# teboli/polyblur

Hardware: AMD Instinct MI355X
Metric: megapixels/sec (n_iter=3, alpha=6, beta=1) (higher is better)
Workload: dtype f32; 1 GPU; batch=1 3840x2160x3 fp32 per GPU, n_iter=3, method=fft (circular), full 25-tap support; mode=resident, images_per_gpu=1, height=2160, width=3840, parallelism=images sharded, no data-path collective

## Files before the change

include/polyblur_hip.h:

```cpp
#ifndef POLYBLUR_HIP_H
#define POLYBLUR_HIP_H

#include <stddef.h>
#include <stdint.h>

#ifdef __cplusplus
extern "C" {
#endif

#define PB_VERSION 200
#define PB_KSIZE 25
#define PB_KRAD 12
#define PB_MAX_ANGLES 13
#define PB_MAX_INTERP 64
#define PB_MAX_PHASES 175

typedef struct pb_ctx pb_ctx;

typedef enum pb_status {
    PB_OK = 0,
    PB_ERR_BADARG = -1,
    PB_ERR_UNSUPPORTED = -2,
    PB_ERR_HIP = -3,
    PB_ERR_NOMEM = -4
// ... 43 lines not shown
    float kx[PB_KSIZE], ky[PB_KSIZE];
    float acorr_y[PB_KSIZE], acorr_x[PB_KSIZE];
    float gtaps[(PB_KSIZE + 1) * 32];
    float gtaps_odd[(PB_KSIZE + 1) * 32];
    int32_t xt_first;
    int32_t xt_exact_rank1;
    float xt_g1[PB_KSIZE];
    int32_t xt_m[PB_KSIZE];
    float xt_wa[PB_KSIZE], xt_wb[PB_KSIZE];
    int32_t nphase[3];
    int32_t phase[PB_MAX_PHASES + 9];
} pb_blur_info;

int pb_version(void);
int pb_create(pb_ctx **out, int device, void *stream);
int pb_destroy(pb_ctx *ctx);
int pb_set_stream(pb_ctx *ctx, void *stream);
int pb_synchronize(pb_ctx *ctx);
const char *pb_last_error_string(pb_ctx *ctx);
void pb_default_options(pb_options *opt);
typedef enum pb_dense_eval { PB_DENSE_STENCIL = 0, PB_DENSE_AUTO = 1 } pb_dense_eval;
int pb_set_dense_eval(pb_ctx *ctx, int mode, int min_phases);
int pb_body_selection(pb_ctx *ctx, int iteration, int *host, int B);
size_t pb_workspace_bytes(pb_ctx *ctx);

int pb_malloc(pb_ctx *ctx, void **dptr, size_t bytes);
int pb_free(pb_ctx *ctx, void *dptr);
int pb_memcpy_h2d(pb_ctx *ctx, void *dst, const void *src, size_t bytes);
int pb_memcpy_d2h(pb_ctx *ctx, void *dst, const void *src, size_t bytes);

int pb_polyblur_batch(pb_ctx *ctx, const void *in, void *out, int dtype,
                      int B, int C, int H, int W, const pb_options *opt,
                      pb_blur_info *host_info);

int pb_u8_deinterleave(pb_ctx *ctx, const unsigned char *hwc, unsigned char *chw, int B, int C, int H, int W);
int pb_u8_interleave(pb_ctx *ctx, const unsigned char *chw, unsigned char *hwc, int B, int C, int H, int W);


int pb_estimate_blur(pb_ctx *ctx, const void *in, int dtype, int B, int C, int H, int W,
                     const pb_options *opt, pb_blur_info *dev_info);

int pb_make_kernels(pb_ctx *ctx, int B, const float *host_sigma, const float *host_rho,
                    const float *host_theta_rad, int support, pb_blur_info *dev_info);
int pb_set_kernels(pb_ctx *ctx, int B, const float *host_taps, int support, pb_blur_info *dev_info);

int pb_make_separable_kernels(pb_ctx *ctx, int B, const pb_blur_info *dev_info, pb_blur_info *dev_sep, int support,
// ... 77 lines not shown
```

polyblur_amd/_capi.py:

```python
from __future__ import annotations

import ctypes as C
import os
import threading

import numpy as np

PB_KSIZE = 25
PB_KSIZE_MAX = 49
PB_MAX_ANGLES = 13
PB_MAX_INTERP = 64
PB_MAX_PHASES = 175

PB_F32, PB_F16, PB_U8 = 0, 1, 2
PB_WRAP, PB_ZERO = 0, 1
PB_PREFILTER_NONE, PB_PREFILTER_BILATERAL, PB_PREFILTER_DOMAIN_TRANSFORM, PB_PREFILTER_NORMALIZED_CONVOLUTION = 0, 1, 2, 3
PB_SUPPORT_FULL, PB_SUPPORT_ADAPTIVE = 0, 1
PB_DENSE_STENCIL, PB_DENSE_AUTO = 0, 1
PB_DENSE_MIN_PHASES = 16
PB_COMM_CHUNK_AUTO = -1

STATUS = {0: "PB_OK", -1: "PB_ERR_BADARG", -2: "PB_ERR_UNSUPPORTED", -3: "PB_ERR_HIP", -4: "PB_ERR_NOMEM"}

SYMBOLS = [
    "pb_version", "pb_create", "pb_destroy", "pb_set_stream", "pb_synchronize", "pb_last_error_string",
    "pb_default_options", "pb_workspace_bytes", "pb_malloc", "pb_free", "pb_memcpy_h2d", "pb_memcpy_d2h",
    "pb_polyblur_batch", "pb_estimate_blur", "pb_make_kernels", "pb_set_kernels", "pb_fourier_gradients",
    "pb_inverse_filter", "pb_convolve2d", "pb_edgetaper", "pb_halo_mask", "pb_dt_recursive_filter",
    "pb_bilateral5", "pb_time_inner_loop", "pb_profile_begin", "pb_profile_end", "pb_extract_patches",
    "pb_overlap_add", "pb_u8_deinterleave", "pb_u8_interleave", "pb_dt_normalized_convolution",
    "pb_fft_length_supported", "pb_make_separable_kernels", "pb_set_dense_eval",
    "pb_body_selection",
    "pb_comm_shard", "pb_comm_unique_id", "pb_comm_init", "pb_comm_destroy", "pb_comm_scatter", "pb_comm_gather",
    "pb_comm_deblur_from_root", "pb_comm_plan_steps", "pb_comm_plan", "pb_comm_set_chunk", "pb_comm_default_chunk",
    "pb_comm_plan_steps_chunked", "pb_comm_plan_chunked",
]
PROF_TAGS = ["conv", "gray", "grad_rows", "grad_cols", "params", "halo", "prefilter", "other", "conv_fused", "conv_fft"]


class pb_options(C.Structure):
    _fields_ = [
        ("n_iter", C.c_int32), ("c", C.c_float), ("b", C.c_float), ("alpha", C.c_float), ("beta", C.c_float),
        ("sigma_s", C.c_float), ("sigma_r", C.c_float), ("q", C.c_float), ("n_angles", C.c_int32),
        ("n_interpolated_angles", C.c_int32), ("remove_halo", C.c_int32), ("edgetaping", C.c_int32),
        ("prefilter", C.c_int32), ("discard_saturation", C.c_int32), ("boundary", C.c_int32),
        ("support", C.c_int32), ("force_theta_deg", C.c_float), ("separable_approx", C.c_int32), ("half_temporaries", C.c_int32), ("ker_size", C.c_int32),
    ]


class pb_blur_info(C.Structure):
    _fields_ = [
        ("gray_min", C.c_float), ("gray_max", C.c_float), ("mags", C.c_float * PB_MAX_ANGLES),
        ("interp", C.c_float * PB_MAX_INTERP), ("i_min", C.c_int32), ("theta", C.c_float),
        ("sigma", C.c_float), ("rho", C.c_float), ("separable", C.c_int32), ("radius", C.c_int32),
        ("kernel", C.c_float * (PB_KSIZE * PB_KSIZE)), ("kx", C.c_float * PB_KSIZE), ("ky", C.c_float * PB_KSIZE),
# ... 58 lines not shown
            "pb_free": (ci, [vp, vp]),
            "pb_memcpy_h2d": (ci, [vp, vp, vp, sz]),
            "pb_memcpy_d2h": (ci, [vp, vp, vp, sz]),
            "pb_polyblur_batch": (ci, [vp, vp, vp, ci, ci, ci, ci, ci, C.POINTER(pb_options), vp]),
            "pb_u8_deinterleave": (ci, [vp, vp, vp, ci, ci, ci, ci]),
            "pb_u8_interleave": (ci, [vp, vp, vp, ci, ci, ci, ci]),
            "pb_estimate_blur": (ci, [vp, vp, ci, ci, ci, ci, ci, C.POINTER(pb_options), vp]),
            "pb_make_kernels": (ci, [vp, ci, fp, fp, fp, ci, vp]),
            "pb_set_kernels": (ci, [vp, ci, fp, ci, vp]),
            "pb_fourier_gradients": (ci, [vp, vp, ci, ci, ci, vp, vp]),
            "pb_inverse_filter": (ci, [vp, vp, vp, ci, ci, ci, ci, ci, vp, cf, cf, ci, ci, ci, vp, vp]),
            "pb_convolve2d": (ci, [vp, vp, vp, ci, ci, ci, ci, vp, ci]),
            "pb_edgetaper": (ci, [vp, vp, vp, ci, ci, ci, ci, vp, ci]),
            "pb_halo_mask": (ci, [vp, vp, vp, vp, vp, vp, ci, ci, ci, ci]),
            "pb_dt_recursive_filter": (ci, [vp, vp, vp, vp, ci, ci, ci, ci, ci, cf, cf, ci]),
            "pb_dt_normalized_convolution": (ci, [vp, vp, vp, ci, ci, ci, ci, ci, cf, cf, ci]),
            "pb_bilateral5": (ci, [vp, vp, vp, ci, ci, ci, ci, ci]),
            "pb_time_inner_loop": (ci, [vp, vp, vp, ci, ci, ci, ci, ci, vp, cf, cf, ci, ci, fp]),
            "pb_extract_patches": (ci, [vp, vp, vp] + [ci] * 15),
            "pb_overlap_add": (ci, [vp, vp, vp] + [ci] * 13 + [vp, vp]),
            "pb_fft_length_supported": (ci, [ci]),
            "pb_make_separable_kernels": (ci, [vp, ci, vp, vp, ci, ci]),
            "pb_body_selection": (ci, [vp, ci, C.POINTER(ci), ci]),
            "pb_profile_begin": (ci, [vp]),
            "pb_profile_end": (ci, [vp, fp, C.POINTER(ci)]),
            "pb_comm_shard": (ci, [ci, ci, ci, C.POINTER(ci), C.POINTER(ci)]),
            "pb_comm_unique_id": (ci, [C.c_char_p]),
            "pb_comm_init": (ci, [C.POINTER(vp), vp, ci, ci, C.c_char_p]),
            "pb_comm_destroy": (ci, [vp]),
            "pb_comm_scatter": (ci, [vp, vp, vp, ci, ci, ci, ci, ci, ci]),
            "pb_comm_gather": (ci, [vp, vp, vp, ci, ci, ci, ci, ci, ci]),
            "pb_comm_deblur_from_root": (ci, [vp, vp, vp, ci, ci, ci, ci, ci, C.POINTER(pb_options), ci]),
            "pb_comm_plan_steps": (ci, [ci, ci, ci]),
            "pb_comm_plan": (ci, [ci, ci, ci, ci, ci, C.POINTER(ci), C.POINTER(ci)]),
            "pb_comm_set_chunk": (ci, [vp, ci]),
            "pb_comm_default_chunk": (ci, [ci, ci, ci]),
            "pb_comm_plan_steps_chunked": (ci, [ci, ci, ci, ci]),
            "pb_comm_plan_chunked": (ci, [ci, ci, ci, ci, ci, ci, C.POINTER(ci), C.POINTER(ci)]),
        }
        for name in SYMBOLS:
            fn = getattr(lib, name)
            fn.restype, fn.argtypes = proto[name]
        _lib = lib
        return lib
```

polyblur_amd/csrc/api.hip:

```cpp
#include <cstdlib>
#include <cstring>

#include "common.h"

int pb_grad_energy(pb_ctx *ctx, const void *gx, const void *gy, float *nM, int P, long HW, int g_dtype = PB_F32);
int pb_halo_apply(pb_ctx *ctx, const void *x, int x_dtype, int x_pitch, long x_plane, const float *y, const void *gx,
                  const void *gy, const void *ox, const float *nM, void *out, int out_dtype, int P, int H, int W,
                  int clamp01, const void *recomb_cur = nullptr, int recomb_cur_dtype = 0, const float *recomb_smooth = nullptr,
                  int g_dtype = PB_F32);
int pb_recombine(pb_ctx *ctx, const float *y, const void *cur, int cur_dtype, const float *smooth, void *out, int out_dtype,
                 long n);
int pb_bilateral5_impl(pb_ctx *ctx, const void *in, int in_dtype, void *out, int out_dtype, int P, int H, int W);
int pb_dt_filter_impl(pb_ctx *ctx, const void *in, const void *joint, int dtype, float *out, int B, int C, int H, int W,
                      float sigma_s, float sigma_r, int num_iterations);
int pb_nc_filter_impl(pb_ctx *ctx, const void *in, int dtype, float *out, int B, int C, int H, int W, float sigma_s,
                      float sigma_r, int num_iterations);
int pb_convert_from_float(pb_ctx *ctx, const float *in, void *out, int dtype, long n);
int pb_u8_layout(pb_ctx *ctx, const unsigned char *in, unsigned char *out, int B, int C, int H, int W, int to_planar);
int pb_convert_to_float(pb_ctx *ctx, const void *in, int dtype, float *out, long n);
int pb_extract_patches_impl(pb_ctx *ctx, const void *img, void *patches, int dtype, int B, int C, int H, int W, int ph, int pw,
                            int step_h, int step_w, int n_j, int pad_top, int pad_left, int first, int count);
int pb_overlap_add_impl(pb_ctx *ctx, const void *patches, void *out, int dtype, int B, int C, int H, int W, int ph, int pw,
                        int step_h, int step_w, int n_i, int n_j, int pad_top, int pad_left, const float *win_y,
                        const float *win_x);
// ... 56 lines not shown
}

extern "C" {

int pb_version(void) { return PB_VERSION; }

void pb_default_options(pb_options *o) {
    memset(o, 0, sizeof(*o));
    o->n_iter = 1; o->c = 0.352f; o->b = 0.768f; o->alpha = 2.f; o->beta = 3.f;
    o->sigma_r = 0.8f; o->sigma_s = 2.0f; o->q = 0.f; o->n_angles = 6; o->n_interpolated_angles = 30;
    o->remove_halo = 0; o->edgetaping = 0; o->prefilter = PB_PREFILTER_NONE; o->discard_saturation = 0;
    o->boundary = PB_WRAP; o->support = PB_SUPPORT_FULL; o->force_theta_deg = -1.f; o->ker_size = PB_KSIZE;
}

int pb_create(pb_ctx **out, int device, void *stream) {
    if (!out) return PB_ERR_BADARG;
    *out = nullptr;
    int n = 0;
    if (hipGetDeviceCount(&n) != hipSuccess || n <= 0 || device < 0 || device >= n) return PB_ERR_HIP;
    if (hipSetDevice(device) != hipSuccess) return PB_ERR_HIP;
    pb_ctx *ctx = new pb_ctx();
    ctx->device = device;
    ctx->stream = static_cast<hipStream_t>(stream);
    pb_read_knobs(ctx);
    if (hipEventCreate(&ctx->ev0) != hipSuccess || hipEventCreate(&ctx->ev1) != hipSuccess ||
        hipEventCreateWithFlags(&ctx->ev_switch, hipEventDisableTiming) != hipSuccess) { delete ctx; return PB_ERR_HIP; }
    {
        if (hipStreamCreateWithFlags(&ctx->aux, hipStreamNonBlocking) != hipSuccess ||
            hipEventCreateWithFlags(&ctx->ev_fork, hipEventDisableTiming) != hipSuccess ||
            hipEventCreateWithFlags(&ctx->ev_join, hipEventDisableTiming) != hipSuccess) {
            (void)hipGetLastError();
            if (ctx->aux) (void)hipStreamDestroy(ctx->aux);
            ctx->aux = nullptr;
        }
    }
    *out = ctx;
    return PB_OK;
}

int pb_set_dense_eval(pb_ctx *ctx, int mode, int min_phases) {
    if (!ctx || (mode != PB_DENSE_STENCIL && mode != PB_DENSE_AUTO) || min_phases < 0 || min_phases > PB_MAX_PHASES + 1)
        return PB_ERR_BADARG;
    ctx->fft_min_phases = mode == PB_DENSE_STENCIL ? -1 : min_phases;
    pb_forget_records(ctx, nullptr, 0);
    return PB_OK;
}
// ... 811 lines not shown
```

polyblur_amd/csrc/common.h:

```cpp
#pragma once
#include <hip/hip_runtime.h>
#include <hip/hip_fp16.h>

#include <cstdarg>
#include <cstdio>
#include <map>
#include <string>
#include <vector>

#include "../../include/polyblur_hip.h"


struct FftPlan {
    int n = 0;
    int nstage = 0;
    int radix[24];
    int bluestein_m = 0;
    float2 *tw = nullptr;
    float *drev = nullptr;
    float2 *chirp = nullptr;
    float2 *bfilt_rev = nullptr;
    float *dnat = nullptr;
};

// ... 1 lines not shown
    void *p = nullptr;
    size_t bytes = 0;
};

struct ProfRec {
    hipEvent_t a, b;
    int tag;
};

struct PolySpec { int on; float a3, a2, a1, b; float gain; int min_area; float cost128; int always; };
inline PolySpec no_poly() { return PolySpec{0, 0.f, 0.f, 0.f, 0.f, 0.f, 0, 0.f, 0}; }
inline bool same_spec(const PolySpec &x, const PolySpec &y) {
    return x.on == y.on && x.always == y.always &&
           (!x.on || (x.a3 == y.a3 && x.a2 == y.a2 && x.a1 == y.a1 && x.b == y.b && (x.cost128 > 0.f) == (y.cost128 > 0.f)));
}

struct pb_fft_sel { int use_fft; int rf; int strip; int poly; int hx; int hy; int pad_[2]; };

struct pb_ctx {
    bool prof_on = false;
    std::vector<ProfRec> prof;
    std::vector<hipEvent_t> evpool;
    int device = 0;
    hipStream_t stream = nullptr;
    std::string err;
    std::map<std::string, ScratchBuf> scratch;
    std::map<int, FftPlan> plans;
    float *interp_w = nullptr;
    int interp_na = 0, interp_ni = 0;
    hipEvent_t ev0 = nullptr, ev1 = nullptr, ev_switch = nullptr;
    hipStream_t aux = nullptr;
    hipEvent_t ev_fork = nullptr, ev_join = nullptr;
    size_t est_done_bytes = 0;
    int fft_min_phases = 16;
    int fft_wave = 1;
    struct BodyFlags { bool any_fft = false, any_other = false, any_strip = false, any_tile = false, any_fft3 = false; };
    struct RecFlags { int B; BodyFlags plain; bool poly_valid; PolySpec spec; BodyFlags poly; std::vector<pb_fft_sel> sel; };
    std::map<const void *, RecFlags> rec_cache;
    struct FlipSet { int B; int support; std::vector<float> taps; };
    std::map<const void *, FlipSet> flip_sets;
    int sel_slot = 0, sel_last = 0, sel_B = 0;
    const std::vector<pb_fft_sel> *known_sel = nullptr;
    const void *khat_owner = nullptr;
    int khat_slot = 0;
    int khat_B = 0;
    const void *khat_buf = nullptr;
// ... 181 lines not shown
```

polyblur_amd/csrc/conv_w128.hip:

```cpp

#include <algorithm>
#include <cstdlib>
#include <type_traits>

#include "conv_wave_common.h"

namespace {

constexpr int W_N = 128;
constexpr int W_P = 129;
constexpr size_t kW128Lds = sizeof(float2) * 64 * W_P;

static __device__ const float kC128[64] = {
    1.0f, 0.9987954497337341f, 0.9951847195625305f, 0.9891765117645264f, 0.9807852506637573f, 0.9700312614440918f,
    0.9569403529167175f, 0.9415440559387207f, 0.9238795042037964f, 0.903989315032959f, 0.8819212913513184f, 0.8577286005020142f,
    0.8314695954322815f, 0.803207516670227f, 0.7730104327201843f, 0.7409511208534241f, 0.7071067690849304f, 0.6715589761734009f,
    0.6343932747840881f, 0.5956993103027344f, 0.5555702447891235f, 0.5141027569770813f, 0.4713967442512512f, 0.4275550842285156f,
    0.3826834261417389f, 0.3368898630142212f, 0.290284663438797f, 0.24298018217086792f, 0.19509032368659973f, 0.1467304676771164f,
    0.0980171412229538f, 0.049067676067352295f, 6.123234262925839e-17f, -0.049067676067352295f, -0.0980171412229538f, -0.1467304676771164f,
    -0.19509032368659973f, -0.24298018217086792f, -0.290284663438797f, -0.3368898630142212f, -0.3826834261417389f, -0.4275550842285156f,
    -0.4713967442512512f, -0.5141027569770813f, -0.5555702447891235f, -0.5956993103027344f, -0.6343932747840881f, -0.6715589761734009f,
    -0.7071067690849304f, -0.7409511208534241f, -0.7730104327201843f, -0.803207516670227f, -0.8314695954322815f, -0.8577286005020142f,
    -0.8819212913513184f, -0.903989315032959f, -0.9238795042037964f, -0.9415440559387207f, -0.9569403529167175f, -0.9700312614440918f,
    -0.9807852506637573f, -0.9891765117645264f, -0.9951847195625305f, -0.9987954497337341f};
// ... 352 lines not shown
            const int row0 = 64 * h;
            const int rlo = max(hy - row0, 0), rhi = min(rmax - row0, 64);
            const unsigned baseA = okA && rlo < rhi ? (unsigned)((wy0 + row0 + rlo - oo) * opitchb + (pxA - oo) * (int)sizeof(TOut)) : kNoAccess;
            const unsigned baseB = okB && rlo < rhi ? (unsigned)((wy0 + row0 + rlo - oo) * opitchb + (pxB - oo) * (int)sizeof(TOut)) : kNoAccess;
#pragma unroll
            for (int r = 0; r < 64; ++r) {
                const bool rok = r >= rlo && r < rhi;
                cf ea = v[r], eb = v[r];
                swap_halves(ea, eb);
                const cf er = ea + eb * sg;
                const float ra = __builtin_amdgcn_fmed3f(er.x, clo, chi), rb = __builtin_amdgcn_fmed3f(er.y, clo, chi);
                BufIO<TOut>::st(ro, rok ? baseA + (unsigned)((r - rlo) * opitchb) : kNoAccess, 0, ra);
                BufIO<TOut>::st(ro, rok ? baseB + (unsigned)((r - rlo) * opitchb) : kNoAccess, 0, rb);
            }
        }
    }
    PB_WT(8);
    PB_WRT(10);
}

template <typename TIn, typename TOut, bool ZERO>
__global__ __launch_bounds__(256, 2) void conv_w128_kernel(const ConvPass a, const W128Geom g) {
    extern __shared__ __attribute__((aligned(16))) float2 Zw[];
    const int lane = threadIdx.x & 63;
#if defined(PB_EXPERIMENTAL) && defined(PB_W128_TRACE)
    unsigned long long *tr = (blockIdx.x < kTraceGroups && threadIdx.x < 64) ? g_w128_trace + (long)blockIdx.x * kTraceStamps : nullptr;
    PB_WT(0);
    PB_WRT(9);
#endif
    const int C = a.C, B = a.P / C;
    const int q = (int)(blockIdx.x & 7u);
    int rem = (int)(blockIdx.x >> 3);
    int img = 0, hx = 0, hy = 0;
    if (B == 1) {
        const PB_CONSTANT pb_fft_sel *s0 = as_constant(a.fsel);
        if (!s0->use_fft || s0->poly != 2) return;
        hx = s0->hx; hy = s0->hy;
    } else {
        auto share_of = [&](int i) -> int {
            if (i >= B) return 0;
            const pb_fft_sel s = a.fsel[i];
            if (!s.use_fft || s.poly != 2) return 0;
            return jobs128_of(g, s.hx, s.hy).per * C;
        };
        bool work = false;
        int base = 0;
        for (int c0 = 0; c0 < B; c0 += 64) {
            const int n = share_of(c0 + lane), incl = wave_scan(n, lane);
            const unsigned long long m = __ballot(base + incl > rem);
            if (m) {
                const int l = __builtin_ctzll(m);
                img = c0 + l;
                rem -= base + (__builtin_amdgcn_readlane(incl, l) - __builtin_amdgcn_readlane(n, l));
                work = true;
                break;
            }
            base += __builtin_amdgcn_readlane(incl, 63);
        }
        if (!work) return;
        img = __builtin_amdgcn_readfirstlane(img); rem = __builtin_amdgcn_readfirstlane(rem);
        hx = as_constant(a.fsel + img)->hx; hy = as_constant(a.fsel + img)->hy;
    }
    const W128Jobs j = jobs128_of(g, hx, hy);
    const int pl = __builtin_amdgcn_readfirstlane(div_rcp128(rem, __builtin_amdgcn_rcpf((float)j.per)));
    if (pl >= C) return;
    const int pair = q * j.per + (rem - pl * j.per);
    if (pair >= j.njobs) return;
    const int ty = __builtin_amdgcn_readfirstlane(div_rcp128(pair, j.inv_pairs_x)), pxi = pair - ty * j.pairs_x;
    w128_pair<TIn, TOut, ZERO>(a, img * C + pl, ty, pxi, hx, hy, Zw, a.khat + (long)img * PB_KHAT_STRIDE PB_WT_PASS);
}

template <typename TIn, typename TOut>
int launch_w128_typed(pb_ctx *ctx, const ConvPass &p, const W128Geom &g, long groups) {
    if (p.boundary == PB_ZERO)
        hipLaunchKernelGGL((conv_w128_kernel<TIn, TOut, true>), dim3((unsigned)groups), dim3(256), kW128Lds, ctx->stream, p, g);
    else
        hipLaunchKernelGGL((conv_w128_kernel<TIn, TOut, false>), dim3((unsigned)groups), dim3(256), kW128Lds, ctx->stream, p, g);
    PB_LAUNCH_CHECK();
    return PB_OK;
}

}

#if defined(PB_EXPERIMENTAL) && defined(PB_W128_TRACE)
extern "C" int pb_debug_w128_trace(unsigned long long *host) {
    int rc = (int)hipMemcpyFromSymbol(host, HIP_SYMBOL(g_w128_trace), sizeof(g_w128_trace));
    static unsigned long long zeros[kTraceGroups * kTraceStamps];
    if (!rc) rc = (int)hipMemcpyToSymbol(HIP_SYMBOL(g_w128_trace), zeros, sizeof(zeros));
    return rc;
}
#endif

bool pb_conv_w128_types(int in_dtype, int out_dtype) { return in_dtype >= 0 && in_dtype <= 2 && out_dtype >= 0 && out_dtype <= 2; }

bool pb_conv_w128_feasible(const ConvPass &p) {
    const int oh = (p.out_kind == OUT_INTERIOR) ? p.H : p.H + 2 * p.pad, ow = (p.out_kind == OUT_INTERIOR) ? p.W : p.W + 2 * p.pad;
    const int t = PB_POLY128_MIN_T;
    const long nj = (long)(((ow + t - 1) / t + 1) / 2) * ((oh + t - 1) / t);
    const long groups = 8L * ((nj + 7) / 8) * p.P;
    return groups > 0 && groups <= (1L << 23);
// ... 41 lines not shown
```

polyblur_amd/csrc/conv_wave_common.h:

```cpp
#pragma once
#include "conv_fft_common.h"

namespace {

constexpr int WF_ROWS = 32;
constexpr size_t kWfLdsWave = sizeof(float2) * WF_ROWS * FT_P;

static __device__ const float kC64[64] = {
    1.0f, 0.9951847195625305f, 0.9807852506637573f, 0.9569403529167175f, 0.9238795042037964f, 0.8819212913513184f,
    0.8314695954322815f, 0.7730104327201843f, 0.7071067690849304f, 0.6343932747840881f, 0.5555702447891235f,
    0.4713967442512512f, 0.3826834261417389f, 0.290284663438797f, 0.19509032368659973f, 0.0980171412229538f, 0.0f,
    -0.0980171412229538f, -0.19509032368659973f, -0.290284663438797f, -0.3826834261417389f, -0.4713967442512512f,
    -0.5555702447891235f, -0.6343932747840881f, -0.7071067690849304f, -0.7730104327201843f, -0.8314695954322815f,
    -0.8819212913513184f, -0.9238795042037964f, -0.9569403529167175f, -0.9807852506637573f, -0.9951847195625305f, -1.0f,
    -0.9951847195625305f, -0.9807852506637573f, -0.9569403529167175f, -0.9238795042037964f, -0.8819212913513184f,
    -0.8314695954322815f, -0.7730104327201843f, -0.7071067690849304f, -0.6343932747840881f, -0.5555702447891235f,
    -0.4713967442512512f, -0.3826834261417389f, -0.290284663438797f, -0.19509032368659973f, -0.0980171412229538f, 0.0f,
    0.0980171412229538f, 0.19509032368659973f, 0.290284663438797f, 0.3826834261417389f, 0.4713967442512512f,
    0.5555702447891235f, 0.6343932747840881f, 0.7071067690849304f, 0.7730104327201843f, 0.8314695954322815f,
    0.8819212913513184f, 0.9238795042037964f, 0.9569403529167175f, 0.9807852506637573f, 0.9951847195625305f};
static __device__ const float kS64[64] = {
    0.0f, 0.0980171412229538f, 0.19509032368659973f, 0.290284663438797f, 0.3826834261417389f, 0.4713967442512512f,
    0.5555702447891235f, 0.6343932747840881f, 0.7071067690849304f, 0.7730104327201843f, 0.8314695954322815f,
    0.8819212913513184f, 0.9238795042037964f, 0.9569403529167175f, 0.9807852506637573f, 0.9951847195625305f, 1.0f,
// ... 89 lines not shown
__device__ __forceinline__ void swap_halves(cf &hi_part, cf &lo_part) {
    typedef unsigned u2 __attribute__((ext_vector_type(2)));
    const u2 x = __builtin_amdgcn_permlane32_swap(__float_as_uint(hi_part.x), __float_as_uint(lo_part.x), false, false);
    const u2 y = __builtin_amdgcn_permlane32_swap(__float_as_uint(hi_part.y), __float_as_uint(lo_part.y), false, false);
    hi_part = (cf){__uint_as_float(x[0]), __uint_as_float(y[0])};
    lo_part = (cf){__uint_as_float(x[1]), __uint_as_float(y[1])};
}

__device__ __forceinline__ void transpose64(cf (&v)[64], float2 *Z, int lane) {
#pragma unroll
    for (int r = 0; r < 32; ++r) swap_halves(v[r], v[32 + r]);
    const float2 *rd = Z + (lane & 31) * FT_P + (lane & 32);
#pragma unroll
    for (int h = 0; h < 2; ++h) {
#pragma unroll
        for (int r = 0; r < 32; ++r) Z[r * FT_P + lane] = pbfft::to_f2(v[32 * h + r]);
        wave_lds_fence();
#pragma unroll
        for (int c = 0; c < 32; ++c) v[32 * h + c] = pbfft::to_cf(rd[c]);
        wave_lds_fence();
    }
}

__device__ __forceinline__ int wave_scan(int x, int lane) {
#pragma unroll
    for (int d = 1; d < 64; d <<= 1) {
        const int t = __shfl_up(x, d, 64);
        if (lane >= d) x += t;
    }
    return x;
}


#pragma clang diagnostic push
#pragma clang diagnostic ignored "-Wold-style-cast"
typedef __attribute__((address_space(3))) void lds_void;
typedef __attribute__((address_space(3))) char lds_char;
__device__ __forceinline__ lds_char *lds_ptr(void *p) { return (lds_char *)p; }
template <int IMM> __device__ __forceinline__ void dma16(brsrc r, lds_char *dst, unsigned voffset, int soffset) {
    __builtin_amdgcn_raw_ptr_buffer_load_lds(r, (lds_void *)dst, 16, (int)voffset, soffset, IMM, 0);
}
#pragma clang diagnostic pop
template <int IMM> __device__ __forceinline__ void dma4(brsrc r, lds_char *dst, unsigned voffset, int soffset) {
    __builtin_amdgcn_raw_ptr_buffer_load_lds(r, (lds_void *)dst, 4, (int)voffset, soffset, IMM, 0);
}
__device__ __forceinline__ void wait_vm0() { asm volatile("s_waitcnt vmcnt(0)" ::: "memory"); }
// ... 50 lines not shown
```

polyblur_amd/csrc/conv_wfft.hip:

```cpp

#include <algorithm>
#include <cstdlib>
#include <type_traits>

#include "conv_wave_common.h"

namespace {

struct WGeom { int ow, oh; };
struct WJobs { int pairs_x, njobs, per; float inv_pairs_x; };
__device__ __forceinline__ int div_rcp(int n, float rcp_d) { return (int)(((float)n + 0.5f) * rcp_d); }
__device__ __forceinline__ WJobs jobs_of(const WGeom &g, int hx, int hy) {
    const int Tx = FT_N - 2 * hx, Ty = FT_N - 2 * hy;
    const int tiles_x = div_rcp(g.ow + Tx - 1, __builtin_amdgcn_rcpf((float)Tx)), tiles_y = div_rcp(g.oh + Ty - 1, __builtin_amdgcn_rcpf((float)Ty));
    WJobs j;
    j.pairs_x = (tiles_x + 1) >> 1;
    j.njobs = j.pairs_x * tiles_y;
    j.per = (j.njobs + 7) >> 3;
    j.inv_pairs_x = __builtin_amdgcn_rcpf((float)j.pairs_x);
    return j;
}

#ifdef PB_WF_TRACE
constexpr int kTraceWaves = 8192, kTraceStamps = 14;
// ... 505 lines not shown
    }
    for (int r = y0; r < y1; ++r)
        for (int c = x0 + lane; c < x1; c += 64)
            pb_st(opl + (long)(r - oo) * a.out_pitch + (c - oo), pb_ld(xpl + (long)(r - xsh) * a.x_pitch + (c - xsh)));
}

__device__ __forceinline__ bool ring_live(const ConvPass &a, int ty, int pxi, int hx, int hy) {
    const int Tx = FT_N - 2 * hx, Ty = FT_N - 2 * hy;
    const OutRegion rg = out_region(a);
    const int Hp = a.H + 2 * a.pad, Wp = a.W + 2 * a.pad;
    const int y0 = rg.y_lo + ty * Ty, y1 = min(y0 + Ty, rg.y_hi), x0 = rg.x_lo + 2 * pxi * Tx, x1 = min(x0 + 2 * Tx, rg.x_hi);
    const int dy = min(y0, Hp - y1), dx = min(x0, Wp - x1);
    if (a.ring >= 4) {
        const int mt = a.ring - 4;
        return dy < 25 + 12 * mt + mt * Ty || dx < 25 + 12 * mt + 2 * mt * Tx;
    }
    const int m = 3 - a.ring;
    return dy < 24 + 12 * m + m * Ty || dx < 24 + 12 * m + 2 * m * Tx;
}

template <typename TIn, typename TX, typename TOut, bool ZERO>
__global__ __launch_bounds__(64, 2) void conv_wfft_kernel(const ConvPass a, const WGeom g) {
    extern __shared__ __attribute__((aligned(16))) char zb[];
    const int lane = threadIdx.x & 63;
    unsigned long long *tr = nullptr;
#ifdef PB_WF_TRACE
    if (blockIdx.x < kTraceWaves) tr = g_wf_trace + (long)blockIdx.x * kTraceStamps;
    PB_T(0);
    PB_TRT(12);
#endif
    const int C = a.C, B = a.P / C;
    const int q = (int)(blockIdx.x & 7u);
    int rem = (int)(blockIdx.x >> 3);
    int img = 0, hx = 0, hy = 0;
    bool fold = false;
    if (B == 1) {
        const PB_CONSTANT pb_fft_sel *s0 = as_constant(a.fsel);
        if (!s0->use_fft || s0->poly == 2 || !poly_match(a.poly, s0->poly)) return;
        hx = s0->hx; hy = s0->hy;
        fold = a.poly == 2 && s0->poly != 0;
    } else {
        auto share_of = [&](int i) -> int {
            if (i >= B) return 0;
            const pb_fft_sel s = a.fsel[i];
            if (!s.use_fft || s.poly == 2 || !poly_match(a.poly, s.poly)) return 0;
            return jobs_of(g, s.hx, s.hy).per * C;
        };
        bool work = false;
        int base = 0;
        for (int c0 = 0; c0 < B; c0 += 64) {
            const int n = share_of(c0 + lane), incl = wave_scan(n, lane);
            const unsigned long long m = __ballot(base + incl > rem);
            if (m) {
                const int l = __builtin_ctzll(m);
                img = c0 + l;
                rem -= base + (__builtin_amdgcn_readlane(incl, l) - __builtin_amdgcn_readlane(n, l));
                work = true;
                break;
            }
            base += __builtin_amdgcn_readlane(incl, 63);
        }
        if (!work) return;
        img = __builtin_amdgcn_readfirstlane(img); rem = __builtin_amdgcn_readfirstlane(rem);
        hx = as_constant(a.fsel + img)->hx; hy = as_constant(a.fsel + img)->hy;
        fold = a.poly == 2 && as_constant(a.fsel + img)->poly != 0;
    }
    const WJobs j = jobs_of(g, hx, hy);
    const int pl = __builtin_amdgcn_readfirstlane(div_rcp(rem, __builtin_amdgcn_rcpf((float)j.per)));
    if (pl >= C) return;
    const int pair = q * j.per + (rem - pl * j.per);
    if (pair >= j.njobs) return;
    const int ty = __builtin_amdgcn_readfirstlane(div_rcp(pair, j.inv_pairs_x)), pxi = pair - ty * j.pairs_x;
    const int plane = img * C + pl;
    const float *kp = a.khat + (long)img * PB_KHAT_STRIDE;
    const pb_blur_info *info = a.info + img;
    if (a.ring && !ring_live(a, ty, pxi, hx, hy)) return;
    const ConvPass af = fold_pass(a, fold);
    if (taper_is_copy(af, ty, pxi, hx, hy)) { copy_pair<TX, TOut>(af, plane, ty, pxi, hx, hy); return; }
    if (pair_is_fast<TIn, TX, TOut>(af, ty, pxi, hx, hy)) wave_pair<1, TIn, TX, TOut, ZERO>(af, info, plane, ty, pxi, hx, hy, zb, kp, tr);
    else if (pair_is_gen<TIn, TX, TOut>(af, pxi, hx)) wave_pair<2, TIn, TX, TOut, ZERO>(af, info, plane, ty, pxi, hx, hy, zb, kp, tr);
    else wave_pair<0, TIn, TX, TOut, ZERO>(af, info, plane, ty, pxi, hx, hy, zb, kp, tr);
}

bool wfft_geometry(const ConvPass &p, bool poly2, float min_area, WGeom &g, long &per_max, long &pairs12) {
    g.oh = (p.out_kind == OUT_INTERIOR) ? p.H : p.H + 2 * p.pad;
    g.ow = (p.out_kind == OUT_INTERIOR) ? p.W : p.W + 2 * p.pad;
    per_max = 0; pairs12 = 0;
    for (int hx = 4; hx <= 28; hx += 4) {
        for (int hy = 2; hy <= 30; hy += 2) {
            const int tx = FT_N - 2 * hx, ty = FT_N - 2 * hy;
            const bool three = hx <= 12 && hy <= 12;
            const bool one = poly2 && tx >= PB_POLY_MIN_TX && ty >= PB_POLY_MIN_TY && (float)(tx * ty) >= min_area;
            if (!three && !one) continue;
            const long nj = (long)(((g.ow + tx - 1) / tx + 1) / 2) * ((g.oh + ty - 1) / ty);
            if (nj > (1L << 20)) return false;
            per_max = std::max(per_max, (nj + 7) / 8);
            if (hx == 12 && hy == 12) pairs12 = nj;
        }
    }
    const long total = 8 * per_max * p.P;
    return total > 0 && total <= (1L << 23);
}

template <typename TIn, typename TX, typename TOut>
int launch_wfft_typed(pb_ctx *ctx, const ConvPass &p, const WGeom &g, long groups) {
    if (p.boundary == PB_ZERO)
        hipLaunchKernelGGL((conv_wfft_kernel<TIn, TX, TOut, true>), dim3((unsigned)groups), dim3(64), kWfLdsWave, ctx->stream, p, g);
    else
        hipLaunchKernelGGL((conv_wfft_kernel<TIn, TX, TOut, false>), dim3((unsigned)groups), dim3(64), kWfLdsWave, ctx->stream, p, g);
    PB_LAUNCH_CHECK();
    return PB_OK;
}

}

#ifdef PB_WF_TRACE
extern "C" int pb_debug_wf_trace_clear(void) {
    void *p = nullptr;
    if (hipGetSymbolAddress(&p, HIP_SYMBOL(g_wf_trace)) != hipSuccess) return -1;
    return (int)hipMemset(p, 0, sizeof(unsigned long long) * kTraceStamps * kTraceWaves);
}
extern "C" int pb_debug_wf_trace(unsigned long long *host, int n_waves) {
    if (n_waves > kTraceWaves) n_waves = kTraceWaves;
    return (int)hipMemcpyFromSymbol(host, HIP_SYMBOL(g_wf_trace), sizeof(unsigned long long) * kTraceStamps * n_waves);
}
#endif

bool pb_conv_wfft_feasible(const ConvPass &p, bool poly2, int min_area) {
    WGeom g; long per_max = 0, pairs12 = 0;
    return wfft_geometry(p, poly2, (float)min_area, g, per_max, pairs12);
}

bool pb_conv_wfft_types(const ConvPass &p) {
    switch (p.in_dtype * 9 + p.x_dtype * 3 + p.out_dtype) {
        case 0: case 1: case 3: case 4: case 12: case 13: case 24: case 26: case 6: case 8: case 2: return true;
        default: return false;
    }
}

int pb_launch_conv_wfft(pb_ctx *ctx, const ConvPass &p) {
    const long min_jobs = ctx->wave_min_jobs;
    if (!pb_conv_wfft_types(p)) return PB_ERR_UNSUPPORTED;
    const bool poly2 = p.poly != 0 && pb_spec_of_spectra(ctx, p.khat).on >= 2;
    const float min_area = (float)ctx->poly_min_area;
    WGeom g;
    long per_max = 0, pairs12 = 0;
    if (!wfft_geometry(p, poly2, min_area, g, per_max, pairs12)) {
        if (poly2) return pb_fail(ctx, PB_ERR_UNSUPPORTED, "conv pass: too many windows for the tile-spectrum body");
        return PB_ERR_UNSUPPORTED;
// ... 36 lines not shown
```

Before: 16870 MP/s.

## Use persistent grid-stride job loops with boundary-first tile ordering in FFT conv kernels

Turns the wfft and w128 conv kernels from one-block-per-job launches into persistent blocks. The grid is sized from the occupancy query times the CU count, and each block strides through the job list. Within each octant, jobs are reordered by slow_first_offset so that the top and bottom edge rows and the left and right edge columns, which take the slower general paths, are issued before interior tiles to even out the tail. The price is per-iteration LDS fences or __syncthreads, a cached per-image prefix table, and extra index math per job.

After: 14840 MP/s (median of 2 runs). -12.1%, worse.

```diff
diff --git a/include/polyblur_hip.h b/include/polyblur_hip.h
--- a/include/polyblur_hip.h
+++ b/include/polyblur_hip.h
@@ -89,6 +89,7 @@
 typedef enum pb_dense_eval { PB_DENSE_STENCIL = 0, PB_DENSE_AUTO = 1 } pb_dense_eval;
 int pb_set_dense_eval(pb_ctx *ctx, int mode, int min_phases);
 int pb_body_selection(pb_ctx *ctx, int iteration, int *host, int B);
+int pb_job_order(int pairs_x, int tiles_y, int q, int r);
 size_t pb_workspace_bytes(pb_ctx *ctx);
 
 int pb_malloc(pb_ctx *ctx, void **dptr, size_t bytes);
diff --git a/polyblur_amd/_capi.py b/polyblur_amd/_capi.py
--- a/polyblur_amd/_capi.py
+++ b/polyblur_amd/_capi.py
@@ -30,7 +30,7 @@
     "pb_bilateral5", "pb_time_inner_loop", "pb_profile_begin", "pb_profile_end", "pb_extract_patches",
     "pb_overlap_add", "pb_u8_deinterleave", "pb_u8_interleave", "pb_dt_normalized_convolution",
     "pb_fft_length_supported", "pb_make_separable_kernels", "pb_set_dense_eval",
-    "pb_body_selection",
+    "pb_body_selection", "pb_job_order",
     "pb_comm_shard", "pb_comm_unique_id", "pb_comm_init", "pb_comm_destroy", "pb_comm_scatter", "pb_comm_gather",
     "pb_comm_deblur_from_root", "pb_comm_plan_steps", "pb_comm_plan", "pb_comm_set_chunk", "pb_comm_default_chunk",
     "pb_comm_plan_steps_chunked", "pb_comm_plan_chunked",
@@ -135,6 +135,7 @@
             "pb_fft_length_supported": (ci, [ci]),
             "pb_make_separable_kernels": (ci, [vp, ci, vp, vp, ci, ci]),
             "pb_body_selection": (ci, [vp, ci, C.POINTER(ci), ci]),
+            "pb_job_order": (ci, [ci, ci, ci, ci]),
             "pb_profile_begin": (ci, [vp]),
             "pb_profile_end": (ci, [vp, fp, C.POINTER(ci)]),
             "pb_comm_shard": (ci, [ci, ci, ci, C.POINTER(ci), C.POINTER(ci)]),
diff --git a/polyblur_amd/csrc/api.hip b/polyblur_amd/csrc/api.hip
--- a/polyblur_amd/csrc/api.hip
+++ b/polyblur_amd/csrc/api.hip
@@ -102,6 +102,7 @@
     pb_ctx *ctx = new pb_ctx();
     ctx->device = device;
     ctx->stream = static_cast<hipStream_t>(stream);
+    if (hipDeviceGetAttribute(&ctx->num_cus, hipDeviceAttributeMultiprocessorCount, device) != hipSuccess) { delete ctx; return PB_ERR_HIP; }
     pb_read_knobs(ctx);
     if (hipEventCreate(&ctx->ev0) != hipSuccess || hipEventCreate(&ctx->ev1) != hipSuccess ||
         hipEventCreateWithFlags(&ctx->ev_switch, hipEventDisableTiming) != hipSuccess) { delete ctx; return PB_ERR_HIP; }
diff --git a/polyblur_amd/csrc/common.h b/polyblur_amd/csrc/common.h
--- a/polyblur_amd/csrc/common.h
+++ b/polyblur_amd/csrc/common.h
@@ -47,6 +47,7 @@
     std::vector<ProfRec> prof;
     std::vector<hipEvent_t> evpool;
     int device = 0;
+    int num_cus = 0;
     hipStream_t stream = nullptr;
     std::string err;
     std::map<std::string, ScratchBuf> scratch;
diff --git a/polyblur_amd/csrc/conv_w128.hip b/polyblur_amd/csrc/conv_w128.hip
--- a/polyblur_amd/csrc/conv_w128.hip
+++ b/polyblur_amd/csrc/conv_w128.hip
@@ -398,60 +398,91 @@
 template <typename TIn, typename TOut, bool ZERO>
 __global__ __launch_bounds__(256, 2) void conv_w128_kernel(const ConvPass a, const W128Geom g) {
     extern __shared__ __attribute__((aligned(16))) float2 Zw[];
+    __shared__ int tab[64];
     const int lane = threadIdx.x & 63;
 #if defined(PB_EXPERIMENTAL) && defined(PB_W128_TRACE)
-    unsigned long long *tr = (blockIdx.x < kTraceGroups && threadIdx.x < 64) ? g_w128_trace + (long)blockIdx.x * kTraceStamps : nullptr;
-    PB_WT(0);
-    PB_WRT(9);
+    unsigned long long *tr = nullptr;
 #endif
     const int C = a.C, B = a.P / C;
-    const int q = (int)(blockIdx.x & 7u);
-    int rem = (int)(blockIdx.x >> 3);
-    int img = 0, hx = 0, hy = 0;
+    const int q = (int)(blockIdx.x & 7u), stride = (int)(gridDim.x >> 3);
+    int pos = (int)(blockIdx.x >> 3);
+    int total = 0, img = 0, img_base = 0, img_end = 0, hx = 0, hy = 0;
+    W128Jobs j = {};
+    auto share_of = [&](int i) -> int {
+        if (i >= B) return 0;
+        const pb_fft_sel s = a.fsel[i];
+        if (!s.use_fft || s.poly != 2) return 0;
+        return jobs128_of(g, s.hx, s.hy).per * C;
+    };
     if (B == 1) {
         const PB_CONSTANT pb_fft_sel *s0 = as_constant(a.fsel);
         if (!s0->use_fft || s0->poly != 2) return;
         hx = s0->hx; hy = s0->hy;
+        j = jobs128_of(g, hx, hy);
+        total = img_end = j.per * C;
+    } else if (B <= 64) {
+        const int incl = wave_scan(share_of(lane), lane);
+        if (threadIdx.x < 64) tab[lane] = incl;
+        __syncthreads();
+        total = __builtin_amdgcn_readlane(incl, 63);
     } else {
-        auto share_of = [&](int i) -> int {
-            if (i >= B) return 0;
-            const pb_fft_sel s = a.fsel[i];
-            if (!s.use_fft || s.poly != 2) return 0;
-            return jobs128_of(g, s.hx, s.hy).per * C;
-        };
-        bool work = false;
-        int base = 0;
-        for (int c0 = 0; c0 < B; c0 += 64) {
-            const int n = share_of(c0 + lane), incl = wave_scan(n, lane);
-            const unsigned long long m = __ballot(base + incl > rem);
-            if (m) {
-                const int l = __builtin_ctzll(m);
-                img = c0 + l;
-                rem -= base + (__builtin_amdgcn_readlane(incl, l) - __builtin_amdgcn_readlane(n, l));
-                work = true;
-                break;
+        for (int c0 = 0; c0 < B; c0 += 64) total += __builtin_amdgcn_readlane(wave_scan(share_of(c0 + lane), lane), 63);
+    }
+    for (; pos < total; pos += stride) {
+#if defined(PB_EXPERIMENTAL) && defined(PB_W128_TRACE)
+        tr = (pos * 8 + q < kTraceGroups && threadIdx.x < 64) ? g_w128_trace + (long)(pos * 8 + q) * kTraceStamps : nullptr;
+        PB_WT(0);
+        PB_WRT(9);
+#endif
+        if (pos >= img_end) {
+            if (B <= 64) {
+                const int incl = tab[lane];
+                const int l = __builtin_ctzll(__ballot(incl > pos));
+                img = l;
+                img_end = __builtin_amdgcn_readlane(incl, l);
+                img_base = l ? __builtin_amdgcn_readlane(incl, l - 1) : 0;
+            } else {
+                int base = 0;
+                for (int c0 = 0; c0 < B; c0 += 64) {
+                    const int n = share_of(c0 + lane), incl = wave_scan(n, lane);
+                    const unsigned long long m = __ballot(base + incl > pos);
+                    if (m) {
+                        const int l = __builtin_ctzll(m);
+                        img = c0 + l;
+                        img_end = base + __builtin_amdgcn_readlane(incl, l);
+                        img_base = img_end - __builtin_amdgcn_readlane(n, l);
+                        break;
+                    }
+                    base += __builtin_amdgcn_readlane(incl, 63);
+                }
             }
-            base += __builtin_amdgcn_readlane(incl, 63);
+            img = __builtin_amdgcn_readfirstlane(img);
+            img_base = __builtin_amdgcn_readfirstlane(img_base); img_end = __builtin_amdgcn_readfirstlane(img_end);
+            hx = as_constant(a.fsel + img)->hx; hy = as_constant(a.fsel + img)->hy;
+            j = jobs128_of(g, hx, hy);
         }
-        if (!work) return;
-        img = __builtin_amdgcn_readfirstlane(img); rem = __builtin_amdgcn_readfirstlane(rem);
-        hx = as_constant(a.fsel + img)->hx; hy = as_constant(a.fsel + img)->hy;
-    }
-    const W128Jobs j = jobs128_of(g, hx, hy);
-    const int pl = __builtin_amdgcn_readfirstlane(div_rcp128(rem, __builtin_amdgcn_rcpf((float)j.per)));
-    if (pl >= C) return;
-    const int pair = q * j.per + (rem - pl * j.per);
-    if (pair >= j.njobs) return;
-    const int ty = __builtin_amdgcn_readfirstlane(div_rcp128(pair, j.inv_pairs_x)), pxi = pair - ty * j.pairs_x;
-    w128_pair<TIn, TOut, ZERO>(a, img * C + pl, ty, pxi, hx, hy, Zw, a.khat + (long)img * PB_KHAT_STRIDE PB_WT_PASS);
+        const int rem = pos - img_base;
+        const int pl = __builtin_amdgcn_readfirstlane(div_rcp128(rem, __builtin_amdgcn_rcpf((float)j.per)));
+        const int tiles_y = __builtin_amdgcn_readfirstlane(div_rcp128(j.njobs, j.inv_pairs_x));
+        const int pair = q * j.per + __builtin_amdgcn_readfirstlane(slow_first_offset(rem - pl * j.per, q, j.pairs_x, tiles_y, j.per));
+        if (pair >= j.njobs) continue;
+        const int ty = __builtin_amdgcn_readfirstlane(div_rcp128(pair, j.inv_pairs_x)), pxi = pair - ty * j.pairs_x;
+        w128_pair<TIn, TOut, ZERO>(a, img * C + pl, ty, pxi, hx, hy, Zw, a.khat + (long)img * PB_KHAT_STRIDE PB_WT_PASS);
+        __syncthreads();
+    }
 }
 
 template <typename TIn, typename TOut>
 int launch_w128_typed(pb_ctx *ctx, const ConvPass &p, const W128Geom &g, long groups) {
-    if (p.boundary == PB_ZERO)
-        hipLaunchKernelGGL((conv_w128_kernel<TIn, TOut, true>), dim3((unsigned)groups), dim3(256), kW128Lds, ctx->stream, p, g);
+    static const int per_cu[2] = {blocks_per_cu(conv_w128_kernel<TIn, TOut, false>, 256, kW128Lds),
+                                  blocks_per_cu(conv_w128_kernel<TIn, TOut, true>, 256, kW128Lds)};
+    const bool zero = p.boundary == PB_ZERO;
+    if (per_cu[zero] <= 0 || ctx->num_cus <= 0) return pb_fail(ctx, PB_ERR_HIP, "conv pass: occupancy query failed");
+    const unsigned grid = (unsigned)job_loop_grid(groups, per_cu[zero], ctx->num_cus);
+    if (zero)
+        hipLaunchKernelGGL((conv_w128_kernel<TIn, TOut, true>), dim3(grid), dim3(256), kW128Lds, ctx->stream, p, g);
     else
-        hipLaunchKernelGGL((conv_w128_kernel<TIn, TOut, false>), dim3((unsigned)groups), dim3(256), kW128Lds, ctx->stream, p, g);
+        hipLaunchKernelGGL((conv_w128_kernel<TIn, TOut, false>), dim3(grid), dim3(256), kW128Lds, ctx->stream, p, g);
     PB_LAUNCH_CHECK();
     return PB_OK;
 }
diff --git a/polyblur_amd/csrc/conv_wave_common.h b/polyblur_amd/csrc/conv_wave_common.h
--- a/polyblur_amd/csrc/conv_wave_common.h
+++ b/polyblur_amd/csrc/conv_wave_common.h
@@ -135,6 +135,44 @@
     }
 }
 
+__host__ __device__ inline int slow_first_offset(int r, int q, int pairs_x, int tiles_y, int per) {
+    const int njobs = pairs_x * tiles_y;
+    const int s = q * per, e = s + per < njobs ? s + per : njobs;
+    if (s + r >= e) return r;
+    const int top_end = pairs_x < njobs ? pairs_x : njobs;
+    const int bot_beg = njobs - pairs_x > top_end ? njobs - pairs_x : top_end;
+    const int n_top = s < top_end ? (e < top_end ? e : top_end) - s : 0;
+    if (r < n_top) return r;
+    r -= n_top;
+    const int bs = s > bot_beg ? s : bot_beg;
+    const int n_bot = e > bs ? e - bs : 0;
+    if (r < n_bot) return bs + r - s;
+    r -= n_bot;
+    const int ms = s > top_end ? s : top_end, me = e < bot_beg ? e : bot_beg;
+    if (pairs_x <= 2) return ms + r - s;
+    const int rows_s = ms / pairs_x, rows_e = me / pairs_x;
+    const int f_s = 2 * rows_s + (ms - rows_s * pairs_x >= 1), f_e = 2 * rows_e + (me - rows_e * pairs_x >= 1);
+    if (r < f_e - f_s) {
+        const int k = f_s + r;
+        return (k >> 1) * pairs_x + ((k & 1) ? pairs_x - 1 : 0) - s;
+    }
+    r -= f_e - f_s;
+    const int k = ms - f_s + r, row = k / (pairs_x - 2);
+    return row * pairs_x + 1 + (k - row * (pairs_x - 2)) - s;
+}
+
+template <typename K> inline int blocks_per_cu(K kernel, int threads, size_t lds_bytes) {
+    int n = 0;
+    if (hipOccupancyMaxActiveBlocksPerMultiprocessor(&n, kernel, threads, lds_bytes) != hipSuccess) { (void)hipGetLastError(); return 0; }
+    return n;
+}
+inline long job_loop_grid(long entries, int blocks_per_cu, int num_cus) {
+    long slots = (long)blocks_per_cu * num_cus;
+    slots -= slots % 8;
+    if (slots < 8) slots = 8;
+    return entries < slots ? entries : slots;
+}
+
 __device__ __forceinline__ int wave_scan(int x, int lane) {
 #pragma unroll
     for (int d = 1; d < 64; d <<= 1) {
diff --git a/polyblur_amd/csrc/conv_wfft.hip b/polyblur_amd/csrc/conv_wfft.hip
--- a/polyblur_amd/csrc/conv_wfft.hip
+++ b/polyblur_amd/csrc/conv_wfft.hip
@@ -551,64 +551,88 @@
 template <typename TIn, typename TX, typename TOut, bool ZERO>
 __global__ __launch_bounds__(64, 2) void conv_wfft_kernel(const ConvPass a, const WGeom g) {
     extern __shared__ __attribute__((aligned(16))) char zb[];
+    __shared__ int tab[64];
     const int lane = threadIdx.x & 63;
     unsigned long long *tr = nullptr;
-#ifdef PB_WF_TRACE
-    if (blockIdx.x < kTraceWaves) tr = g_wf_trace + (long)blockIdx.x * kTraceStamps;
-    PB_T(0);
-    PB_TRT(12);
-#endif
     const int C = a.C, B = a.P / C;
-    const int q = (int)(blockIdx.x & 7u);
-    int rem = (int)(blockIdx.x >> 3);
-    int img = 0, hx = 0, hy = 0;
+    const int q = (int)(blockIdx.x & 7u), stride = (int)(gridDim.x >> 3);
+    int pos = (int)(blockIdx.x >> 3);
+    int total = 0, img = 0, img_base = 0, img_end = 0, hx = 0, hy = 0;
     bool fold = false;
+    WJobs j = {};
+    auto share_of = [&](int i) -> int {
+        if (i >= B) return 0;
+        const pb_fft_sel s = a.fsel[i];
+        if (!s.use_fft || s.poly == 2 || !poly_match(a.poly, s.poly)) return 0;
+        return jobs_of(g, s.hx, s.hy).per * C;
+    };
     if (B == 1) {
         const PB_CONSTANT pb_fft_sel *s0 = as_constant(a.fsel);
         if (!s0->use_fft || s0->poly == 2 || !poly_match(a.poly, s0->poly)) return;
         hx = s0->hx; hy = s0->hy;
         fold = a.poly == 2 && s0->poly != 0;
+        j = jobs_of(g, hx, hy);
+        total = img_end = j.per * C;
+    } else if (B <= 64) {
+        const int incl = wave_scan(share_of(lane), lane);
+        tab[lane] = incl;
+        wave_lds_fence();
+        total = __builtin_amdgcn_readlane(incl, 63);
     } else {
-        auto share_of = [&](int i) -> int {
-            if (i >= B) return 0;
-            const pb_fft_sel s = a.fsel[i];
-            if (!s.use_fft || s.poly == 2 || !poly_match(a.poly, s.poly)) return 0;
-            return jobs_of(g, s.hx, s.hy).per * C;
-        };
-        bool work = false;
-        int base = 0;
-        for (int c0 = 0; c0 < B; c0 += 64) {
-            const int n = share_of(c0 + lane), incl = wave_scan(n, lane);
-            const unsigned long long m = __ballot(base + incl > rem);
-            if (m) {
-                const int l = __builtin_ctzll(m);
-                img = c0 + l;
-                rem -= base + (__builtin_amdgcn_readlane(incl, l) - __builtin_amdgcn_readlane(n, l));
-                work = true;
-                break;
-            }
-            base += __builtin_amdgcn_readlane(incl, 63);
-        }
-        if (!work) return;
-        img = __builtin_amdgcn_readfirstlane(img); rem = __builtin_amdgcn_readfirstlane(rem);
-        hx = as_constant(a.fsel + img)->hx; hy = as_constant(a.fsel + img)->hy;
-        fold = a.poly == 2 && as_constant(a.fsel + img)->poly != 0;
-    }
-    const WJobs j = jobs_of(g, hx, hy);
-    const int pl = __builtin_amdgcn_readfirstlane(div_rcp(rem, __builtin_amdgcn_rcpf((float)j.per)));
-    if (pl >= C) return;
-    const int pair = q * j.per + (rem - pl * j.per);
-    if (pair >= j.njobs) return;
-    const int ty = __builtin_amdgcn_readfirstlane(div_rcp(pair, j.inv_pairs_x)), pxi = pair - ty * j.pairs_x;
-    const int plane = img * C + pl;
-    const float *kp = a.khat + (long)img * PB_KHAT_STRIDE;
-    const pb_blur_info *info = a.info + img;
-    if (a.ring && !ring_live(a, ty, pxi, hx, hy)) return;
-    const ConvPass af = fold_pass(a, fold);
-    if (taper_is_copy(af, ty, pxi, hx, hy)) { copy_pair<TX, TOut>(af, plane, ty, pxi, hx, hy); return; }
-    if (pair_is_fast<TIn, TX, TOut>(af, ty, pxi, hx, hy)) wave_pair<1, TIn, TX, TOut, ZERO>(af, info, plane, ty, pxi, hx, hy, zb, kp, tr);
-    else if (pair_is_gen<TIn, TX, TOut>(af, pxi, hx)) wave_pair<2, TIn, TX, TOut, ZERO>(af, info, plane, ty, pxi, hx, hy, zb, kp, tr);
-    else wave_pair<0, TIn, TX, TOut, ZERO>(af, info, plane, ty, pxi, hx, hy, zb, kp, tr);
+        for (int c0 = 0; c0 < B; c0 += 64) total += __builtin_amdgcn_readlane(wave_scan(share_of(c0 + lane), lane), 63);
+    }
+    for (; pos < total; pos += stride) {
+#ifdef PB_WF_TRACE
+        tr = pos * 8 + q < kTraceWaves ? g_wf_trace + (long)(pos * 8 + q) * kTraceStamps : nullptr;
+        PB_T(0);
+        PB_TRT(12);
+#endif
+        if (pos >= img_end) {
+            if (B <= 64) {
+                const int incl = tab[lane];
+                const int l = __builtin_ctzll(__ballot(incl > pos));
+                img = l;
+                img_end = __builtin_amdgcn_readlane(incl, l);
+                img_base = l ? __builtin_amdgcn_readlane(incl, l - 1) : 0;
+            } else {
+                int base = 0;
+                for (int c0 = 0; c0 < B; c0 += 64) {
+                    const int n = share_of(c0 + lane), incl = wave_scan(n, lane);
+                    const unsigned long long m = __ballot(base + incl > pos);
+                    if (m) {
+                        const int l = __builtin_ctzll(m);
+                        img = c0 + l;
+                        img_end = base + __builtin_amdgcn_readlane(incl, l);
+                        img_base = img_end - __builtin_amdgcn_readlane(n, l);
+                        break;
+                    }
+                    base += __builtin_amdgcn_readlane(incl, 63);
+                }
+            }
+            img = __builtin_amdgcn_readfirstlane(img);
+            img_base = __builtin_amdgcn_readfirstlane(img_base); img_end = __builtin_amdgcn_readfirstlane(img_end);
+            hx = as_constant(a.fsel + img)->hx; hy = as_constant(a.fsel + img)->hy;
+            fold = a.poly == 2 && as_constant(a.fsel + img)->poly != 0;
+            j = jobs_of(g, hx, hy);
+        }
+        const int rem = pos - img_base;
+        const int pl = __builtin_amdgcn_readfirstlane(div_rcp(rem, __builtin_amdgcn_rcpf((float)j.per)));
+        const int tiles_y = __builtin_amdgcn_readfirstlane(div_rcp(j.njobs, j.inv_pairs_x));
+        const int pair = q * j.per + __builtin_amdgcn_readfirstlane(slow_first_offset(rem - pl * j.per, q, j.pairs_x, tiles_y, j.per));
+        if (pair >= j.njobs) continue;
+        const int ty = __builtin_amdgcn_readfirstlane(div_rcp(pair, j.inv_pairs_x)), pxi = pair - ty * j.pairs_x;
+        const int plane = img * C + pl;
+        const float *kp = a.khat + (long)img * PB_KHAT_STRIDE;
+        const pb_blur_info *info = a.info + img;
+        if (a.ring && !ring_live(a, ty, pxi, hx, hy)) continue;
+        const ConvPass af = fold_pass(a, fold);
+        if (taper_is_copy(af, ty, pxi, hx, hy)) { copy_pair<TX, TOut>(af, plane, ty, pxi, hx, hy); continue; }
+        if (pair_is_fast<TIn, TX, TOut>(af, ty, pxi, hx, hy)) wave_pair<1, TIn, TX, TOut, ZERO>(af, info, plane, ty, pxi, hx, hy, zb, kp, tr);
+        else if (pair_is_gen<TIn, TX, TOut>(af, pxi, hx)) wave_pair<2, TIn, TX, TOut, ZERO>(af, info, plane, ty, pxi, hx, hy, zb, kp, tr);
+        else wave_pair<0, TIn, TX, TOut, ZERO>(af, info, plane, ty, pxi, hx, hy, zb, kp, tr);
+        wait_lds0();
+        wave_lds_fence();
+    }
 }
 
 bool wfft_geometry(const ConvPass &p, bool poly2, float min_area, WGeom &g, long &per_max, long &pairs12) {
@@ -633,10 +657,15 @@
 
 template <typename TIn, typename TX, typename TOut>
 int launch_wfft_typed(pb_ctx *ctx, const ConvPass &p, const WGeom &g, long groups) {
-    if (p.boundary == PB_ZERO)
-        hipLaunchKernelGGL((conv_wfft_kernel<TIn, TX, TOut, true>), dim3((unsigned)groups), dim3(64), kWfLdsWave, ctx->stream, p, g);
+    static const int per_cu[2] = {blocks_per_cu(conv_wfft_kernel<TIn, TX, TOut, false>, 64, kWfLdsWave),
+                                  blocks_per_cu(conv_wfft_kernel<TIn, TX, TOut, true>, 64, kWfLdsWave)};
+    const bool zero = p.boundary == PB_ZERO;
+    if (per_cu[zero] <= 0 || ctx->num_cus <= 0) return pb_fail(ctx, PB_ERR_HIP, "conv pass: occupancy query failed");
+    const unsigned grid = (unsigned)job_loop_grid(groups, per_cu[zero], ctx->num_cus);
+    if (zero)
+        hipLaunchKernelGGL((conv_wfft_kernel<TIn, TX, TOut, true>), dim3(grid), dim3(64), kWfLdsWave, ctx->stream, p, g);
     else
-        hipLaunchKernelGGL((conv_wfft_kernel<TIn, TX, TOut, false>), dim3((unsigned)groups), dim3(64), kWfLdsWave, ctx->stream, p, g);
+        hipLaunchKernelGGL((conv_wfft_kernel<TIn, TX, TOut, false>), dim3(grid), dim3(64), kWfLdsWave, ctx->stream, p, g);
     PB_LAUNCH_CHECK();
     return PB_OK;
 }
@@ -654,6 +683,13 @@
     return (int)hipMemcpyFromSymbol(host, HIP_SYMBOL(g_wf_trace), sizeof(unsigned long long) * kTraceStamps * n_waves);
 }
 #endif
+
+extern "C" int pb_job_order(int pairs_x, int tiles_y, int q, int r) {
+    if (pairs_x < 1 || tiles_y < 1 || (long)pairs_x * tiles_y > (1L << 20) || q < 0 || q > 7) return -1;
+    const int per = (pairs_x * tiles_y + 7) >> 3;
+    if (r < 0 || r >= per) return -1;
+    return slow_first_offset(r, q, pairs_x, tiles_y, per);
+}
 
 bool pb_conv_wfft_feasible(const ConvPass &p, bool poly2, int min_area) {
     WGeom g; long per_max = 0, pairs12 = 0;
```
